# alanross/AlvaAR

Measured on NVIDIA H100. Metric: frames_per_sec_720p_1000orb_20kf_ba, higher is better.
Workload: dtype u8/f64

## Files before the change

alvaar_b200/csrc/ba.cu:

```cuda
#include "alva_common.cuh"
#include "../../include/alva_b200.h"
#include <math.h>
#include <float.h>
#include <string.h>

namespace {

constexpr int NMAX = 128;
constexpr int LIN_THREADS = 128;
constexpr int NBMAX = NMAX / 6;
constexpr int MAXKEYS = NBMAX * (NBMAX + 1) / 2;
constexpr int BS_THREADS = 128;

struct BaState {
    double radius, decrease_factor, x_cost, cand_cost, xnorm, gmax, model_change;
    double se_min, se_cur, se_ref, se_cand, se_acc_ref, se_acc_cand;
    double initial_cost, push_cost;
    int reuse_diagonal, invalid_steps, iteration, last_success, n_success, n_iter, term, done;
    int relin, step_ok, ncols, chol_ok;
    int use_gather, nb, nbad, has_last;
    int skipped, pad0;
};

struct BaProblem {
// ... 722 lines not shown
        double av[4], bv[4];
#pragma unroll
        for (int t = 0; t < 4; t++) { av[t] = __ldg(row + i0 + 8 * t + cc); bv[t] = __ldg(row + j0 + 8 * t + cc); }
#pragma unroll
        for (int a = 0; a < 4; a++)
#pragma unroll
            for (int b = 0; b < 4; b++) dmma_m8n8k4(acc[a][b][0], acc[a][b][1], av[a], bv[b]);
    }
#pragma unroll
    for (int a = 0; a < 4; a++)
#pragma unroll
        for (int b = 0; b < 4; b++) {
            part[warp][8 * a + cc][8 * b + 2 * kr] = acc[a][b][0];
            part[warp][8 * a + cc][8 * b + 2 * kr + 1] = acc[a][b][1];
        }
    __syncthreads();
    for (int t = threadIdx.x; t < 32 * 32; t += 128) {
        const int r = t >> 5, c = t & 31;
        const double v = part[0][r][c] + part[1][r][c] + part[2][r][c] + part[3][r][c];
        if (v != 0.0) atomicAdd(&P.S[(i0 + r) * NMAX + j0 + c], -v);
    }
}


__device__ __forceinline__ void lm_landmark(const BaProblem& P, int l) {
    const int b = P.lm_start[l], e = P.lm_start[l + 1];
    if (e == b) return;
    const int ca = P.pose_col[P.anch_kf[l]];
    const double sce = P.sce[l];
    double ete = P.De[l] * P.De[l], etb = 0, wa[6] = {0, 0, 0, 0, 0, 0};
    for (int i = b; i < e; i++) {
        const int o = P.lm_obs[i];
        const int cp = P.pose_col[P.obs_kf[o]];
        const double e0 = P.Jd[2 * o] * sce, e1 = P.Jd[2 * o + 1] * sce;
        ete += e0 * e0 + e1 * e1;
        etb += e0 * P.res[2 * o] + e1 * P.res[2 * o + 1];
        for (int c = 0; c < 6; c++) {
            if (ca >= 0) wa[c] += (e0 * P.Ja[12 * o + c] + e1 * P.Ja[12 * o + 6 + c]) * P.scf[ca + c];
            P.wp[6 * o + c] = cp >= 0 ? (e0 * -P.Ja[12 * o + c] + e1 * -P.Ja[12 * o + 6 + c]) * P.scf[cp + c] : 0.0;
        }
    }
    P.ete[l] = ete;
    P.etb[l] = etb;
    for (int c = 0; c < 6; c++) P.wa[6 * l + c] = wa[c];
}
__global__ void __launch_bounds__(128) ba_lm_kernel(const BaProblem* __restrict__ probs, BaDims D) {
    const BaProblem P = probs[blockIdx.y];
    if (P.st->done) return;
    const int l = blockIdx.x * 128 + threadIdx.x;
    if (P.st->use_gather) { if (l < D.nlm) lm_landmark(P, l); }
    else if (l < D.nlm) schur_landmark<false>(P, D, l);
}

template <bool TRANSPOSE>
__device__ __forceinline__ void gather_entry(const BaProblem& P, uint64_t en, const double* sci, const double* scj, double* acc,
                                             double* rh) {
    const int l = (int)(en >> 48), su = (int)(en >> 40) & 0xff, sv = (int)(en >> 32) & 0xff;
    const double inv = 1.0 / P.ete[l], etb = P.etb[l];
    const int ou = su ? (int)(en >> 16) & 0xffff : -1, ov = sv ? (int)en & 0xffff : -1;
    double wu[6], wv[6];
#pragma unroll
    for (int c = 0; c < 6; c++) {
        wu[c] = (su ? P.wp[6 * ou + c] : P.wa[6 * l + c]) * inv;
        wv[c] = sv ? P.wp[6 * ov + c] : P.wa[6 * l + c];
    }
#define ACC(a, c) acc[TRANSPOSE ? 6 * (c) + (a) : 6 * (a) + (c)]
#pragma unroll
    for (int a = 0; a < 6; a++)
#pragma unroll
        for (int c = 0; c < 6; c++) ACC(a, c) -= wu[a] * wv[c];
    if (su == 0 && sv == 0) {
        const int ob = P.lm_start[l], oe = P.lm_start[l + 1];
        for (int i = ob; i < oe; i++) {
            const int o = P.lm_obs[i];
            double F0[6], F1[6];
#pragma unroll
            for (int c = 0; c < 6; c++) { F0[c] = P.Ja[12 * o + c] * sci[c]; F1[c] = P.Ja[12 * o + 6 + c] * sci[c]; }
            const double r0 = P.res[2 * o], r1 = P.res[2 * o + 1];
#pragma unroll
            for (int a = 0; a < 6; a++) {
                if (!TRANSPOSE) rh[a] += F0[a] * r0 + F1[a] * r1;
#pragma unroll
                for (int c = 0; c < 6; c++) ACC(a, c) += F0[a] * F0[c] + F1[a] * F1[c];
            }
        }
        if (!TRANSPOSE)
#pragma unroll
            for (int a = 0; a < 6; a++) rh[a] -= wu[a] * etb;
    } else if (su == sv) {
        double F0[6], F1[6];
#pragma unroll
        for (int c = 0; c < 6; c++) { F0[c] = -P.Ja[12 * ou + c] * sci[c]; F1[c] = -P.Ja[12 * ou + 6 + c] * sci[c]; }
        const double r0 = P.res[2 * ou], r1 = P.res[2 * ou + 1];
#pragma unroll
        for (int a = 0; a < 6; a++) {
            if (!TRANSPOSE) rh[a] += F0[a] * r0 + F1[a] * r1 - wu[a] * etb;
#pragma unroll
            for (int c = 0; c < 6; c++) ACC(a, c) += F0[a] * F0[c] + F1[a] * F1[c];
        }
    } else if (su == 0 || sv == 0) {
        const int o = su ? ou : ov;
        double A0[6], A1[6];
#pragma unroll
        for (int a = 0; a < 6; a++) {
            A0[a] = (su ? -P.Ja[12 * o + a] : P.Ja[12 * o + a]) * sci[a];
            A1[a] = (su ? -P.Ja[12 * o + 6 + a] : P.Ja[12 * o + 6 + a]) * sci[a];
        }
#pragma unroll
        for (int c = 0; c < 6; c++) {
            const double b0 = (sv ? -P.Ja[12 * o + c] : P.Ja[12 * o + c]) * scj[c];
            const double b1 = (sv ? -P.Ja[12 * o + 6 + c] : P.Ja[12 * o + 6 + c]) * scj[c];
#pragma unroll
            for (int a = 0; a < 6; a++) ACC(a, c) += A0[a] * b0 + A1[a] * b1;
        }
    }
#undef ACC
}

constexpr int GA_THREADS = 64, GA_SPLIT = 8;
constexpr int GA_GRID = NBMAX * GA_SPLIT + (MAXKEYS - NBMAX);
__global__ void __launch_bounds__(GA_THREADS, 8) ba_gather_kernel(const BaProblem* __restrict__ probs, BaDims D) {
    const BaProblem P = probs[blockIdx.y];
    const BaState& st = *P.st;
    if (st.done || !st.use_gather) return;
    int bi, bj, part = 0, nparts = 1;
    if ((int)blockIdx.x < NBMAX * GA_SPLIT) { bi = bj = blockIdx.x / GA_SPLIT; part = blockIdx.x % GA_SPLIT; nparts = GA_SPLIT; }
    else {
        int rem = blockIdx.x - NBMAX * GA_SPLIT;
        bi = 0;
        while (bi < NBMAX - 1 && rem >= NBMAX - 1 - bi) { rem -= NBMAX - 1 - bi; bi++; }
        bj = bi + 1 + rem;
    }
    if (bi >= st.nb || bj >= st.nb) return;
    const int blk = bi * NBMAX + bj;
    __shared__ double red[GA_THREADS / 32][42];
    __shared__ int last_s;
    const int tid = threadIdx.x, lane = tid & 31, warp = tid >> 5;
    const int ci = 6 * bi, cj = 6 * bj;
    const int eb = P.blk_off[blk], ee = eb + P.blk_start[blk + 1];
    double acc[36], rh[6];
#pragma unroll
    for (int i = 0; i < 36; i++) acc[i] = 0.0;
#pragma unroll
    for (int i = 0; i < 6; i++) rh[i] = 0.0;
    double sci[6], scj[6];
#pragma unroll
    for (int c = 0; c < 6; c++) { sci[c] = P.scf[ci + c]; scj[c] = P.scf[cj + c]; }
    for (int idx = eb + part * GA_THREADS + tid; idx < ee; idx += nparts * GA_THREADS) {
        const uint64_t en = P.pairs[idx];
        gather_entry<false>(P, en, sci, scj, acc, rh);
    }
#pragma unroll
    for (int i = 0; i < 36; i++) {
#pragma unroll
        for (int off = 16; off; off >>= 1) acc[i] += __shfl_xor_sync(0xffffffffu, acc[i], off);
        if (lane == 0) red[warp][i] = acc[i];
    }
#pragma unroll
    for (int i = 0; i < 6; i++) {
#pragma unroll
        for (int off = 16; off; off >>= 1) rh[i] += __shfl_xor_sync(0xffffffffu, rh[i], off);
        if (lane == 0) red[warp][36 + i] = rh[i];
    }
    __syncthreads();
    if (nparts > 1) {
        double* slot = P.ga_part + ((size_t)bi * GA_SPLIT + part) * 42;
        for (int x = tid; x < 42; x += GA_THREADS) {
            double v = 0;
#pragma unroll
            for (int wv = 0; wv < GA_THREADS / 32; wv++) v += red[wv][x];
            slot[x] = v;
        }
        __threadfence();
        __syncthreads();
        if (tid == 0) last_s = atomicInc(reinterpret_cast<unsigned int*>(P.ga_ticket + bi), GA_SPLIT - 1) == GA_SPLIT - 1;
        __syncthreads();
        if (!last_s) return;
        __threadfence();
    }
    for (int x = tid; x < 42; x += GA_THREADS) {
        double v = 0;
        if (nparts > 1) {
            const volatile double* all = P.ga_part + (size_t)bi * GA_SPLIT * 42;
#pragma unroll
            for (int q = 0; q < GA_SPLIT; q++) v += all[q * 42 + x];
        } else {
#pragma unroll
            for (int wv = 0; wv < GA_THREADS / 32; wv++) v += red[wv][x];
        }
        if (x < 36) {
            const int a = x / 6, c = x % 6;
            if (bi == bj) P.S[(ci + a) * NMAX + ci + c] = v + (a == c ? P.Df[ci + a] * P.Df[ci + a] : 0.0);
            else { P.S[(ci + a) * NMAX + cj + c] = v; P.S[(cj + c) * NMAX + ci + a] = v; }
        } else if (bi == bj) P.rhs[ci + x - 36] = v;
    }
}

constexpr int CH_TILES = 32 * 33 / 2, CH_THREADS = (CH_TILES + 31) / 32 * 32;
__device__ void ba_chol_body(const BaProblem& P, double* sm) {
    BaState& st = *P.st;
    const int n = st.ncols, tid = threadIdx.x, lane = tid & 31;
    const int ld = NMAX + 1;
    double* V = sm;
    double* invd = sm + NMAX * ld;
    __shared__ double pcol[4][NMAX];
    __shared__ double dg[4][4];
    __shared__ double pivinv[2][4];
    __shared__ int ok_s;
    int tj = 0, rem = tid;
    while (tj < 32 && rem >= 32 - tj) { rem -= 32 - tj; tj++; }
    const int ti = tj + rem;
    const bool tile = tid < CH_TILES;
    const int r0 = 4 * ti, c0 = 4 * tj;
    double a[4][4];
#pragma unroll
// ... 370 lines not shown
    mix((uint64_t)(uintptr_t)obs_lm); mix((uint64_t)(uintptr_t)obs_uv); mix((uint64_t)(uintptr_t)flags);
    if (key != ctx->ba_table_key) {
        std::string hostbuf(sizeof(BaProblem) * nprob, '\0');
        BaProblem* hp = reinterpret_cast<BaProblem*>(&hostbuf[0]);
        for (int p = 0; p < nprob; p++) {
            BaProblem& P = hp[p];
            P.calib = calib + 4 * (size_t)p; P.poses = poses + 7 * (size_t)nkf * p; P.pose_const = pose_const + (size_t)nkf * p;
            P.invd = invd + (size_t)nlm * p; P.anch_kf = anch_kf + (size_t)nlm * p; P.anch_uv = anch_uv + 2 * (size_t)nlm * p;
            P.obs_kf = obs_kf + (size_t)nobs * p; P.obs_lm = obs_lm + (size_t)nobs * p; P.obs_uv = obs_uv + 2 * (size_t)nobs * p;
            double* d = reinterpret_cast<double*>(ws + tab + per * p);
            auto take = [&](size_t n) { double* r = d; d += n; return r; };
            P.res = take(2 * (size_t)nobs); P.Ja = take(12 * (size_t)nobs); P.Jd = take(2 * (size_t)nobs);
            P.wp = take(6 * (size_t)nobs);
            P.nf = take(NMAX); P.gf = take(NMAX); P.scf = take(NMAX); P.diagf = take(NMAX); P.Df = take(NMAX);
            P.ne = take(nlm); P.ge = take(nlm); P.sce = take(nlm); P.diage = take(nlm); P.De = take(nlm);
            P.ete = take(nlm); P.etb = take(nlm); P.wa = take(6 * (size_t)nlm); P.ye = take(nlm);
            P.S = take((size_t)NMAX * NMAX); P.rhs = take(NMAX); P.yf = take(NMAX);
            P.cand_poses = take(7 * (size_t)nkf); P.cand_invd = take(nlm); P.cost_part = take(nblk);
            P.Wt = g_ba_dense_schur ? take((size_t)((nlm + 3) / 4 * 4) * NMAX) : nullptr;
            P.mc_part = take((size_t)((nlm + BS_THREADS - 1) / BS_THREADS));
            P.ga_part = take((size_t)NBMAX * GA_SPLIT * 42);
            P.last_poses = local ? take(7 * (size_t)nkf) : nullptr;
            P.last_invd = local ? take(nlm) : nullptr;
            uint8_t* b = reinterpret_cast<uint8_t*>(d);
            P.pose_col = reinterpret_cast<int32_t*>(b); b += align_up((size_t)nkf * 4, 8);
            P.lm_start = reinterpret_cast<int32_t*>(b); b += align_up((size_t)(nlm + 1) * 4, 8);
            P.lm_obs = reinterpret_cast<int32_t*>(b); b += align_up((size_t)nobs * 4, 8);
            P.obs_col = reinterpret_cast<int32_t*>(b); b += align_up((size_t)nobs * 4, 8);
            P.anch_col = reinterpret_cast<int32_t*>(b); b += align_up((size_t)nlm * 4, 8);
            P.pstart = reinterpret_cast<int32_t*>(b); b += align_up((size_t)(NBMAX + 1) * 4, 8);
            P.plist = reinterpret_cast<uint32_t*>(b); b += align_up(((size_t)nobs + (size_t)nlm) * 4, 8);
            P.blk_start = reinterpret_cast<int32_t*>(b); b += align_up((size_t)(NBMAX * NBMAX + 1) * 4, 8);
            P.blk_off = reinterpret_cast<int32_t*>(b); b += align_up((size_t)(NBMAX * NBMAX + 1) * 4, 8);
            P.pairs = reinterpret_cast<uint64_t*>(b); b += align_up((size_t)(8 * (size_t)nobs + 2 * (size_t)nlm) * 8, 8);
            P.ga_ticket = reinterpret_cast<int32_t*>(b); b += align_up((size_t)NBMAX * 4, 8);
            P.obs_lm_in = nullptr; P.obs_lm_w = nullptr; P.flags = nullptr;
            if (local) {
                P.obs_lm_in = P.obs_lm;
                P.obs_lm_w = reinterpret_cast<int32_t*>(b); b += align_up((size_t)nobs * 4, 8);
                P.obs_lm = P.obs_lm_w;
                P.flags = flags + (size_t)nobs * p;
            }
            P.st = reinterpret_cast<BaState*>(b);
        }
        ALVA_CUDA(cudaMemcpyAsync(ws, hp, sizeof(BaProblem) * nprob, cudaMemcpyHostToDevice, ctx->stream));
        ALVA_CUDA(cudaStreamSynchronize(ctx->stream));
        ctx->ba_table_key = key;
    }
    *dp_out = reinterpret_cast<const BaProblem*>(ws);
    *D_out = BaDims{nkf, nlm, nobs, nblk, 0.0, 0, (nlm + 3) / 4 * 4, 8 * nobs + 2 * nlm, (nlm + BS_THREADS - 1) / BS_THREADS, 0};
    return 0;
}

static int ba_run_solve(alva_ctx* ctx, const BaProblem* dp, const BaDims& D, int nprob) {
    const bool dense = g_ba_dense_schur != 0;
    const size_t chol_smem = ((size_t)NMAX * (NMAX + 1) + NMAX) * sizeof(double);
    ALVA_CUDA(cudaFuncSetAttribute(ba_chol_kernel, cudaFuncAttributeMaxDynamicSharedMemorySize, (int)chol_smem));
    ba_setup_kernel<<<nprob, SETUP_THREADS, 0, ctx->stream>>>(dp, D);
    ALVA_LAUNCH_CHECK(ctx);
    const dim3 lin_grid(D.nblk, nprob), schur_grid((D.nlm_pad + 127) / 128, nprob), syrk_grid(16, SYRK_KSPLIT, nprob);
    const dim3 key_grid(GA_GRID, nprob), bs_grid(D.nbs, nprob), stats_grid(D.nbs + NBMAX, nprob);
    bool forked = false;
    if (!dense) {
        const dim3 pr_grid(NBMAX, nprob);
        cudaStream_t ps = ctx->stream;
        if (ctx->aux_stream && cudaEventRecord(ctx->aux_fork, ctx->stream) == cudaSuccess &&
            cudaStreamWaitEvent(ctx->aux_stream, ctx->aux_fork, 0) == cudaSuccess) { ps = ctx->aux_stream; forked = true; }
        ba_pairs_kernel<0><<<pr_grid, 32, 0, ps>>>(dp, D);
        ALVA_LAUNCH_CHECK(ctx);
        ba_pairs_kernel<1><<<pr_grid, 32, 0, ps>>>(dp, D);
        ALVA_LAUNCH_CHECK(ctx);
        if (forked) ALVA_CUDA(cudaEventRecord(ctx->aux_join, ps));
    }
    for (int it = 0; it <= D.max_iter; it++) {
        ba_linearize_kernel<true><<<lin_grid, LIN_THREADS, 0, ctx->stream>>>(dp, D);
        ALVA_LAUNCH_CHECK(ctx);
        ba_stats_kernel<<<stats_grid, BS_THREADS, 0, ctx->stream>>>(dp, D);
        ALVA_LAUNCH_CHECK(ctx);
        ba_pre_kernel<<<nprob, g_ba_ctl_threads, 0, ctx->stream>>>(dp, D);
        ALVA_LAUNCH_CHECK(ctx);
        if (it == D.max_iter) {
            if (forked) { ALVA_CUDA(cudaStreamWaitEvent(ctx->stream, ctx->aux_join, 0)); forked = false; }
            break;
        }
        if (dense) {
            ba_schur_kernel<true><<<schur_grid, 128, 0, ctx->stream>>>(dp, D);
            ALVA_LAUNCH_CHECK(ctx);
            ba_syrk_dmma_kernel<<<syrk_grid, 128, 0, ctx->stream>>>(dp, D);
            ALVA_LAUNCH_CHECK(ctx);
        } else {
            if (forked) { ALVA_CUDA(cudaStreamWaitEvent(ctx->stream, ctx->aux_join, 0)); forked = false; }
            ba_lm_kernel<<<schur_grid, 128, 0, ctx->stream>>>(dp, D);
            ALVA_LAUNCH_CHECK(ctx);
            ba_gather_kernel<<<key_grid, GA_THREADS, 0, ctx->stream>>>(dp, D);
            ALVA_LAUNCH_CHECK(ctx);
        }
        ba_chol_kernel<<<nprob, CH_THREADS, chol_smem, ctx->stream>>>(dp, D);
        ALVA_LAUNCH_CHECK(ctx);
        ba_backsub_kernel<<<bs_grid, BS_THREADS, 0, ctx->stream>>>(dp, D);
        ALVA_LAUNCH_CHECK(ctx);
        ba_linearize_kernel<false><<<lin_grid, LIN_THREADS, 0, ctx->stream>>>(dp, D);
        ALVA_LAUNCH_CHECK(ctx);
        ba_post_kernel<<<nprob, g_ba_ctl_threads, 0, ctx->stream>>>(dp, D);
        ALVA_LAUNCH_CHECK(ctx);
    }
    return 0;
}

static bool ba_args_ok(alva_ctx* ctx, int nprob, int nkf, int nlm, int nobs, const void* calib, const void* poses,
                       const void* pose_const, const void* invd, const void* anch_kf, const void* anch_uv, const void* obs_kf,
                       const void* obs_lm, const void* obs_uv, int max_iter) {
    return ctx && nprob >= 1 && nkf >= 1 && nkf <= 256 && nlm >= 1 && nobs >= 1 && calib && poses && pose_const && invd &&
           anch_kf && anch_uv && obs_kf && obs_lm && obs_uv && max_iter >= 0;
}

extern "C" int alva_k_ba_solve(alva_ctx* ctx, int nprob, int nkf, int nlm, int nobs, const double* calib, double* poses,
                               const uint8_t* pose_const, double* invd, const int32_t* anch_kf, const double* anch_uv,
                               const int32_t* obs_kf, const int32_t* obs_lm, const double* obs_uv, double huber_delta,
                               int max_iter, double* summary) { AlvaDeviceGuard guard__(ctx);
    if (!ba_args_ok(ctx, nprob, nkf, nlm, nobs, calib, poses, pose_const, invd, anch_kf, anch_uv, obs_kf, obs_lm, obs_uv, max_iter)) {
        alva_set_error("alva_k_ba_solve: bad argument (need 1 <= nkf <= 256)");
        return ALVA_E_INVALID;
    }
    const BaProblem* dp;
    BaDims D;
    if (int e = ba_prepare(ctx, nprob, nkf, nlm, nobs, calib, poses, pose_const, invd, anch_kf, anch_uv, obs_kf, obs_lm, obs_uv,
                           nullptr, &dp, &D))
        return e;
    D.huber = huber_delta; D.max_iter = max_iter;
    if (int e = ba_run_solve(ctx, dp, D, nprob)) return e;
    if (summary) {
        ba_summary_kernel<<<nprob, 32, 0, ctx->stream>>>(dp, summary);
        ALVA_LAUNCH_CHECK(ctx);
    }
    return 0;
}

extern "C" int alva_k_ba_local(alva_ctx* ctx, int nprob, int nkf, int nlm, int nobs, const double* calib, double* poses,
                               const uint8_t* pose_const, double* invd, const int32_t* anch_kf, const double* anch_uv,
                               const int32_t* obs_kf, const int32_t* obs_lm, const double* obs_uv, double huber_delta,
                               double chi2_thr, int max_iter, int32_t* flags, double* summary) { AlvaDeviceGuard guard__(ctx);
    if (!ba_args_ok(ctx, nprob, nkf, nlm, nobs, calib, poses, pose_const, invd, anch_kf, anch_uv, obs_kf, obs_lm, obs_uv, max_iter) ||
        !flags) {
        alva_set_error("alva_k_ba_local: bad argument (need 1 <= nkf <= 256, flags != NULL)");
        return ALVA_E_INVALID;
    }
    const BaProblem* dp;
    BaDims D;
    if (int e = ba_prepare(ctx, nprob, nkf, nlm, nobs, calib, poses, pose_const, invd, anch_kf, anch_uv, obs_kf, obs_lm, obs_uv,
                           flags, &dp, &D))
        return e;
    D.huber = huber_delta; D.max_iter = max_iter;
    const dim3 obs_grid(D.nblk, nprob);
    ba_local_init_kernel<<<obs_grid, LIN_THREADS, 0, ctx->stream>>>(dp, D);
    ALVA_LAUNCH_CHECK(ctx);
    if (int e = ba_run_solve(ctx, dp, D, nprob)) return e;
    if (summary) { ba_summary_local_kernel<<<nprob, 32, 0, ctx->stream>>>(dp, summary, 0); ALVA_LAUNCH_CHECK(ctx); }
    ba_flag_kernel<1><<<obs_grid, LIN_THREADS, 0, ctx->stream>>>(dp, D, chi2_thr);
    ALVA_LAUNCH_CHECK(ctx);
    D.pass = 1; D.max_iter = 5;
    if (int e = ba_run_solve(ctx, dp, D, nprob)) return e;
    ba_flag_kernel<2><<<obs_grid, LIN_THREADS, 0, ctx->stream>>>(dp, D, chi2_thr);
    ALVA_LAUNCH_CHECK(ctx);
    if (summary) { ba_summary_local_kernel<<<nprob, 32, 0, ctx->stream>>>(dp, summary, 1); ALVA_LAUNCH_CHECK(ctx); }
    return 0;
}

extern "C" int alva_k_ba_linearize(alva_ctx* ctx, int nkf, int nlm, int nobs, const double* calib, const double* poses,
                                   const double* invd, const int32_t* anch_kf, const double* anch_uv, const int32_t* obs_kf,
                                   const int32_t* obs_lm, const double* obs_uv, double huber_delta, double* res, double* Ja,
                                   double* Jp, double* Jd, double* cost_per_obs) { AlvaDeviceGuard guard__(ctx);
    if (!ctx || nobs < 1 || !calib || !poses || !invd || !res || !Ja || !Jp || !Jd || !cost_per_obs) {
        alva_set_error("alva_k_ba_linearize: bad argument");
        return ALVA_E_INVALID;
    }
    (void)nkf; (void)nlm;
    ba_linearize_dump_kernel<<<(nobs + 127) / 128, 128, 0, ctx->stream>>>(calib, poses, invd, anch_kf, anch_uv, obs_kf, obs_lm,
                                                                         obs_uv, nobs, huber_delta, res, Ja, Jp, Jd, cost_per_obs);
    ALVA_LAUNCH_CHECK(ctx);
    return 0;
}

extern int alva_g_knn_qpw;
int alva_g_ba_overlap = 1;

extern int alva_g_frontend_antipodal, alva_g_frontend_variant, alva_g_frontend_prefetch, alva_g_frontend_ctas;
extern int alva_g_knn_mma, alva_g_knn_mma_mode, alva_g_knn_mma_kind;
extern int alva_g_pipeline_graphs, alva_g_ba_lag;
extern "C" int alva_set_option(const char* name, int value) {
    if (name && !strcmp(name, "ba_dense_schur")) { g_ba_dense_schur = value ? 1 : 0; return 0; }
    if (name && !strcmp(name, "ba_ctl_threads") && (value == 256 || value == 512 || value == 1024)) { g_ba_ctl_threads = value; return 0; }
    if (name && !strcmp(name, "frontend_antipodal")) { alva_g_frontend_antipodal = value ? 1 : 0; return 0; }
    if (name && !strcmp(name, "frontend_variant") && (value == 0 || value == 2)) { alva_g_frontend_variant = value; return 0; }
    if (name && !strcmp(name, "frontend_ctas") && (value == 4 || value == 5)) { alva_g_frontend_ctas = value; return 0; }
    if (name && !strcmp(name, "frontend_prefetch")) { alva_g_frontend_prefetch = value ? 1 : 0; return 0; }
    if (name && !strcmp(name, "pipeline_graphs")) { alva_g_pipeline_graphs = value ? 1 : 0; return 0; }
    if (name && !strcmp(name, "pipeline_ba_lag")) { alva_g_ba_lag = value ? 1 : 0; return 0; }
    if (name && !strcmp(name, "pipeline_ba_overlap")) { alva_g_ba_overlap = value ? 1 : 0; return 0; }
    if (name && !strcmp(name, "knn_qpw") && (value == 4 || value == 8)) { alva_g_knn_qpw = value; return 0; }
    if (name && !strcmp(name, "knn_mma") && value >= 0 && value <= 2) { alva_g_knn_mma = value; return 0; }
    if (name && !strcmp(name, "knn_mma_kind") && (value == 0 || value == 1)) { alva_g_knn_mma_kind = value; return 0; }
    if (name && !strcmp(name, "knn_mma_mode") && value >= 0 && value <= 2) { alva_g_knn_mma_mode = value; return 0; }
    alva_set_error("alva_set_option: unknown option");
    return ALVA_E_INVALID;
}
```

alvaar_b200/lib.py:

```python
import ctypes as C
import os

_HERE = os.path.dirname(os.path.abspath(__file__))
ORB_FMA = 1
ORB_IC_ANGLE = 2
ORB_HARRIS = 4


class AlvaError(RuntimeError):
    pass


def lib_path():
    return os.path.join(_HERE, "libalva_b200.so")


_lib = None


def lib():
    global _lib
    if _lib is None:
        p = lib_path()
        if not os.path.exists(p):
# ... 1 lines not shown
                            "(there is no CPU fallback)")
        L = C.CDLL(p)
        vp, i32, i64 = C.c_void_p, C.c_int, C.c_longlong
        L.alva_version.restype = i32
        L.alva_last_error.restype = C.c_char_p
        L.alva_ctx_create.restype = vp
        L.alva_ctx_create.argtypes = [i32, vp]
        L.alva_ctx_destroy.argtypes = [vp]
        L.alva_ctx_sync.argtypes = [vp]
        L.alva_ctx_launches.restype = i64
        L.alva_ctx_launches.argtypes = [vp]
        L.alva_k_gray.argtypes = [vp, vp, vp, i32, i32, i32]
        L.alva_k_pyrdown.argtypes = [vp, vp, vp, i32, i32, i32]
        L.alva_k_fast9.argtypes = [vp, vp, i32, i32, i32, i32, vp, vp, i32, i32]
        L.alva_k_frontend.argtypes = [vp, vp, i32, i32, i32, vp, vp, vp, vp, i32, vp, vp, i32, i32]
        L.alva_set_option.argtypes = [C.c_char_p, i32]
        L.alva_k_retain_best.argtypes = [vp, vp, vp, i32, i32, i32, i32, i32, i32, vp, vp, i32]
        for name, args in _OPTIONAL.items():
            if hasattr(L, name):
                getattr(L, name).argtypes = args
        _lib = L
    return _lib


_vp, _i32 = C.c_void_p, C.c_int
_OPTIONAL = {
    "alva_k_orb_blur": [_vp, _vp, _vp, _i32, _i32, _i32, _i32],
    "alva_k_orb_describe": [_vp, _vp, _vp, _i32, _i32, _i32, _vp, _vp, _i32, _i32, _vp, _vp, _vp],
    "alva_k_hamming_knn2": [_vp, _vp, _i32, _vp, _i32, _vp],
    "alva_k_hamming_knn2_batch": [_vp, _vp, _vp, _i32, _i32, _vp, _i32, _vp],
    "alva_h_frontend": [_vp, _vp, _i32, _i32, _i32, _i32, _vp, _vp, _i32],
    "alva_k_scharr": [_vp, _vp, _vp, _i32, _i32, _i32],
    "alva_k_clahe": [_vp, _vp, _vp, _i32, _i32, _i32, C.c_double, _i32, _i32],
    "alva_k_detect_grid": [_vp, _vp, _i32, _i32, _i32, _i32, _vp, _vp, _i32, _vp, _vp, _vp, _vp, _vp, _i32],
    "alva_k_corner_subpix": [_vp, _vp, _i32, _i32, _i32, _vp, _vp, _i32],
    "alva_k_match_to_map": [_vp, _i32, _i32, _i32, C.c_double, C.c_double, C.c_double, C.c_double, _vp, _i32, _vp, _vp, _i32, _i32, _vp,
                            _i32, _vp, _vp, _vp, _vp, _vp, _vp, _vp, _i32, _vp, C.c_float, C.c_float, _vp, _vp, _vp],
    "alva_k_match_to_map_dist": [_vp, _i32, _i32, _i32, C.c_double, C.c_double, C.c_double, C.c_double, _vp, _i32, _vp, _vp, _i32, _i32,
                                 _vp, _i32, _vp, _vp, _vp, _vp, _vp, _vp, _vp, _i32, _vp, C.c_float, C.c_float, _vp, _vp, _vp, _vp],
    "alva_k_undistort_points": [_vp, _vp, _vp, _i32, _i32, _vp, _vp, _vp],
    "alva_k_project_points": [_vp, _vp, _i32, _vp, _vp, _vp],
    "alva_k_p3p_lmeds": [_vp, _i32, _i32, _vp, _vp, _vp, _i32, C.c_float, C.c_float, C.c_float, C.c_uint32, _vp, _vp, _vp],
    "alva_k_pnp": [_vp, _i32, _i32, _vp, _vp, _vp, _vp, _vp, C.c_double, C.c_double, _i32, _i32, _i32, _vp, _vp],
    "alva_k_essential_5pt": [_vp, _i32, _i32, _vp, _vp, _vp, _i32, C.c_float, _i32, C.c_float, C.c_float, C.c_uint32, _vp, _vp, _vp],
    "alva_k_triangulate": [_vp, _vp, _vp, _vp, _i32, _vp],
    "alva_k_klt_lk": [_vp, _vp, _vp, _vp, _i32, _i32, _i32, _i32, _i32, _i32, _i32, C.c_double, _i32, _vp, _vp, _vp, _i32, _vp, _vp],
    "alva_k_klt_fb": [_vp, _vp, _vp, _vp, _vp, _i32, _i32, _i32, _i32, _i32, _i32, C.c_float, C.c_float, _vp, _vp, _vp, _i32, _vp],
    "alva_k_harris": [_vp, _vp, _i32, _i32, _i32, _vp, _vp, _i32, _vp],
    "alva_k_orb_detect": [_vp, _vp, _i32, _i32, _i32, _i32, _i32, _i32, _vp, _vp, _vp, _i32],
    "alva_k_ba_solve": [_vp, _i32, _i32, _i32, _i32, _vp, _vp, _vp, _vp, _vp, _vp, _vp, _vp, _vp, C.c_double, _i32, _vp],
    "alva_k_ba_local": [_vp, _i32, _i32, _i32, _i32, _vp, _vp, _vp, _vp, _vp, _vp, _vp, _vp, _vp, C.c_double, C.c_double,
                        _i32, _vp, _vp],
    "alva_k_ba_linearize": [_vp, _i32, _i32, _i32, _vp, _vp, _vp, _vp, _vp, _vp, _vp, _vp, C.c_double, _vp, _vp, _vp, _vp, _vp],
}


def key_x(k):
    return (k >> 8) & 0xFFF


def key_y(k):
    return (k >> 20) & 0xFFF


def key_score(k):
    return k & 0xFF


def unpack_keys(keys):
    import numpy as np
    k = np.asarray(keys).astype(np.int64) & 0xFFFFFFFF
    return np.stack([(k >> 8) & 0xFFF, (k >> 20) & 0xFFF, k & 0xFF], -1).astype(np.int32)


def _ptr(t):
    if t is None:
        return None
    return C.c_void_p(t.data_ptr())


def _f64x4(v):
    return (C.c_double * 4)(*[float(x) for x in v])


class Context:

    def __init__(self, device=0, stream=None):
        self.L = lib()
        if stream is not None and int(stream) == 0:
            stream = 1
        h = self.L.alva_ctx_create(int(device), C.c_void_p(int(stream)) if stream is not None else None)
        if not h:
            raise AlvaError(self.L.alva_last_error().decode())
        self.h = C.c_void_p(h)
        self.device = device

    def close(self):
        if getattr(self, "h", None):
            self.L.alva_ctx_destroy(self.h)
            self.h = None

    def __del__(self):
        try:
            self.close()
        except Exception:
            pass
# ... 78 lines not shown
                _ptr(kp_match), _ptr(kp_dist), _ptr(n_match))
        if dist is None:
            self._chk(self.L.alva_k_match_to_map(*args))
        else:
            self._chk(self.L.alva_k_match_to_map_dist(*args, _f64x4(dist)))

    def undistort_points(self, px, counts, nframes, cap, K, dist, unpx):
        self._chk(self.L.alva_k_undistort_points(self.h, _ptr(px), _ptr(counts), nframes, cap, _f64x4(K), _f64x4(dist), _ptr(unpx)))

    def project_points(self, Xc, n, K, dist, uv):
        self._chk(self.L.alva_k_project_points(self.h, _ptr(Xc), n, _f64x4(K), _f64x4(dist), _ptr(uv)))

    def p3p_lmeds(self, nprob, cap, bvs, wpts, counts, Twc_out, outlier, info=None, max_iter=100, err_px=3.0, fx=1.0, fy=1.0,
                  seed=12345):
        self._chk(self.L.alva_k_p3p_lmeds(self.h, nprob, cap, _ptr(bvs), _ptr(wpts), _ptr(counts), max_iter, err_px, fx, fy,
                                          seed, _ptr(Twc_out), _ptr(outlier), _ptr(info)))

    def essential_5pt(self, nprob, cap, bv1, bv2, counts, Rt_out, outlier, info=None, max_iter=100, err_px=3.0, optimize=True,
                      fx=1.0, fy=1.0, seed=12345):
        self._chk(self.L.alva_k_essential_5pt(self.h, nprob, cap, _ptr(bv1), _ptr(bv2), _ptr(counts), max_iter, err_px,
                                              int(optimize), fx, fy, seed, _ptr(Rt_out), _ptr(outlier), _ptr(info)))

    def triangulate(self, Tlr, bvl, bvr, n, out):
        self._chk(self.L.alva_k_triangulate(self.h, _ptr(Tlr), _ptr(bvl), _ptr(bvr), n, _ptr(out)))

    def pnp(self, nprob, cap, K, uv, X, counts, poses, outlier, summary, huber_delta, chi2_thr, max_iter=5, use_robust=True,
            apply_l2=True):
        self._chk(self.L.alva_k_pnp(self.h, nprob, cap, _ptr(K), _ptr(uv), _ptr(X), _ptr(counts), _ptr(poses), huber_delta,
                                    chi2_thr, max_iter, 1 if use_robust else 0, 1 if apply_l2 else 0, _ptr(outlier),
                                    _ptr(summary)))

    def hamming_knn2_batch(self, q, counts, nbatch, qcap, t, nt, out):
        self._chk(self.L.alva_k_hamming_knn2_batch(self.h, _ptr(q), _ptr(counts), nbatch, qcap, _ptr(t), nt, _ptr(out)))

    def harris(self, gray, w, h, nframes, pts, npts_per_frame, npts, resp):
        self._chk(self.L.alva_k_harris(self.h, _ptr(gray), w, h, nframes, _ptr(pts), _ptr(npts_per_frame), npts, _ptr(resp)))

    def orb_detect(self, gray, w, h, nframes, nfeatures, fast_thr, flags, kp_out, desc, counts, out_cap):
        self._chk(self.L.alva_k_orb_detect(self.h, _ptr(gray), w, h, nframes, nfeatures, fast_thr, flags, _ptr(kp_out),
                                           _ptr(desc), _ptr(counts), out_cap))

    def ba_solve(self, nprob, nkf, nlm, nobs, calib, poses, pose_const, invd, anch_kf, anch_uv, obs_kf, obs_lm, obs_uv,
                 huber, max_iter, summary=None):
        self._chk(self.L.alva_k_ba_solve(self.h, nprob, nkf, nlm, nobs, _ptr(calib), _ptr(poses), _ptr(pose_const), _ptr(invd),
                                         _ptr(anch_kf), _ptr(anch_uv), _ptr(obs_kf), _ptr(obs_lm), _ptr(obs_uv), huber,
                                         max_iter, _ptr(summary)))

    def ba_local(self, nprob, nkf, nlm, nobs, calib, poses, pose_const, invd, anch_kf, anch_uv, obs_kf, obs_lm, obs_uv,
                 huber, chi2_thr, max_iter, flags, summary=None):
        self._chk(self.L.alva_k_ba_local(self.h, nprob, nkf, nlm, nobs, _ptr(calib), _ptr(poses), _ptr(pose_const), _ptr(invd),
                                         _ptr(anch_kf), _ptr(anch_uv), _ptr(obs_kf), _ptr(obs_lm), _ptr(obs_uv), huber,
                                         chi2_thr, max_iter, _ptr(flags), _ptr(summary)))

    def ba_linearize(self, nkf, nlm, nobs, calib, poses, invd, anch_kf, anch_uv, obs_kf, obs_lm, obs_uv, huber, res, Ja, Jp,
                     Jd, cost):
        self._chk(self.L.alva_k_ba_linearize(self.h, nkf, nlm, nobs, _ptr(calib), _ptr(poses), _ptr(invd), _ptr(anch_kf),
                                             _ptr(anch_uv), _ptr(obs_kf), _ptr(obs_lm), _ptr(obs_uv), huber, _ptr(res),
                                             _ptr(Ja), _ptr(Jp), _ptr(Jd), _ptr(cost)))
```

include/alva_b200.h:

```cpp
#ifndef ALVA_B200_H
#define ALVA_B200_H
#include <stdint.h>
#include <stddef.h>

#ifdef __cplusplus
extern "C" {
#endif

#define ALVA_OK            0
#define ALVA_E_INVALID    -1
#define ALVA_E_CUDA       -2
#define ALVA_E_CAPACITY   -3
#define ALVA_E_STATE      -4

#define ALVA_KEY_X(k)     (((k) >> 8) & 0xFFFu)
#define ALVA_KEY_Y(k)     (((k) >> 20) & 0xFFFu)
#define ALVA_KEY_SCORE(k) ((k) & 0xFFu)
#define ALVA_MAX_DIM      4095

#define ALVA_ORB_FMA        1
#define ALVA_ORB_HARRIS     4
#define ALVA_ORB_IC_ANGLE   2

typedef struct alva_ctx alva_ctx;
// ... 56 lines not shown
int alva_k_klt_lk(alva_ctx*, const uint8_t* const* prev_img, const int16_t* const* prev_der, const uint8_t* const* cur_img,
                  int w, int h, int nframes, int pyr_levels, int levels, int win, int max_count, double epsilon,
                  int use_initial, const float* pts, float* next, const int32_t* npts_per_frame, int npts,
                  uint8_t* status, float* err);

int alva_k_klt_fb(alva_ctx*, const uint8_t* const* prev_img, const int16_t* const* prev_der, const uint8_t* const* cur_img,
                  const int16_t* const* cur_der, int w, int h, int nframes, int pyr_levels, int levels, int win,
                  float error_value, float max_fb_dist, const float* pts, float* priors, const int32_t* npts_per_frame,
                  int npts, uint8_t* good);

int alva_k_p3p_lmeds(alva_ctx*, int nprob, int cap, const double* bvs, const double* wpts, const int32_t* counts,
                     int max_iter, float err_px, float fx, float fy, uint32_t seed, double* Twc_out, uint8_t* outlier,
                     double* info);

int alva_k_pnp(alva_ctx*, int nprob, int cap, const double* K, const double* uv, const double* X, const int32_t* counts,
               double* poses, double huber_delta, double chi2_thr, int max_iter, int use_robust, int apply_l2,
               uint8_t* outlier, double* summary);

int alva_k_essential_5pt(alva_ctx*, int nprob, int cap, const double* bv1, const double* bv2, const int32_t* counts,
                         int max_iter, float err_px, int optimize, float fx, float fy, uint32_t seed, double* Rt_out,
                         uint8_t* outlier, double* info);

int alva_k_triangulate(alva_ctx*, const double* Tlr, const double* bvl, const double* bvr, int n, double* out);

int alva_k_match_to_map(alva_ctx*, int w, int h, int cell, double fx, double fy, double cx, double cy, const double* Twc_cur,
                        int n_kp, const int32_t* kp_mp, const float* kp_px, int nkp3d, int n_kf, const double* kf_Twc, int n_mp,
                        const double* mp_wpt, const uint8_t* mp_is3d, const int32_t* obs_start, const int32_t* obs_kf,
                        const float* obs_px, const int32_t* desc_start, const uint8_t* desc, int n_local, const int32_t* local_mp,
                        float max_proj_err, float dist_ratio, int32_t* kp_match, float* kp_dist, int32_t* n_match);
int alva_k_match_to_map_dist(alva_ctx*, int w, int h, int cell, double fx, double fy, double cx, double cy, const double* Twc_cur,
                             int n_kp, const int32_t* kp_mp, const float* kp_px, int nkp3d, int n_kf, const double* kf_Twc, int n_mp,
                             const double* mp_wpt, const uint8_t* mp_is3d, const int32_t* obs_start, const int32_t* obs_kf,
                             const float* obs_px, const int32_t* desc_start, const uint8_t* desc, int n_local, const int32_t* local_mp,
                             float max_proj_err, float dist_ratio, int32_t* kp_match, float* kp_dist, int32_t* n_match,
                             const double* dist4);

int alva_k_ba_solve(alva_ctx*, int nprob, int nkf, int nlm, int nobs, const double* calib, double* poses,
                    const uint8_t* pose_const, double* invd, const int32_t* anch_kf, const double* anch_uv,
                    const int32_t* obs_kf, const int32_t* obs_lm, const double* obs_uv, double huber_delta, int max_iter,
                    double* summary);

int alva_k_ba_local(alva_ctx*, int nprob, int nkf, int nlm, int nobs, const double* calib, double* poses,
                    const uint8_t* pose_const, double* invd, const int32_t* anch_kf, const double* anch_uv,
                    const int32_t* obs_kf, const int32_t* obs_lm, const double* obs_uv, double huber_delta, double chi2_thr,
                    int max_iter, int32_t* flags, double* summary);

int alva_set_option(const char* name, int value);
int alva_debug_knn2_mma(alva_ctx*, const uint8_t* q, int nq, const uint8_t* t, int nt, int32_t* out, int32_t* dbg_dev);

int alva_k_ba_linearize(alva_ctx*, int nkf, int nlm, int nobs, const double* calib, const double* poses, const double* invd,
                        const int32_t* anch_kf, const double* anch_uv, const int32_t* obs_kf, const int32_t* obs_lm,
                        const double* obs_uv, double huber_delta, double* res, double* Ja, double* Jp, double* Jd,
                        double* cost_per_obs);

typedef struct alva_pipeline alva_pipeline;
typedef struct alva_pipeline_config {
    int w, h, batch;
    int fast_thr;
    int nfeatures;
    int orb_flags;
    int map_size;
    int kf_interval;
    int ba_nkf, ba_nlm, ba_nobs, ba_max_iter;
    double ba_huber;
    int derivatives;
    int reserved;
} alva_pipeline_config;

alva_pipeline* alva_pipeline_create(alva_ctx*, const alva_pipeline_config*);
void alva_pipeline_destroy(alva_pipeline*);
int  alva_pipeline_set_map(alva_pipeline*, const uint8_t* desc_host, int n);
int  alva_pipeline_set_ba(alva_pipeline*, int slot, const double* calib, const double* poses, const uint8_t* pose_const,
                          const double* invd, const int32_t* anch_kf, const double* anch_uv, const int32_t* obs_kf,
                          const int32_t* obs_lm, const double* obs_uv);
int  alva_pipeline_step_dev(alva_pipeline*, const uint8_t* rgba_dev);
int  alva_pipeline_step_host(alva_pipeline*, const uint8_t* rgba_host, int32_t* nfeat_host, int32_t* matches_host,
                             double* ba_poses_host, double* ba_summary_host);
int  alva_pipeline_submit_host(alva_pipeline*, const uint8_t* rgba_host, int32_t* nfeat_host, int32_t* matches_host,
                               double* ba_poses_host, double* ba_summary_host);
int  alva_pipeline_wait(alva_pipeline*);
int  alva_pipeline_profile(alva_pipeline*, int enable);
int  alva_pipeline_frontend_ms(alva_pipeline*, float* ms, int n);
int  alva_pipeline_info(const alva_pipeline*, int32_t* out4);
int  alva_pipeline_graph_stats(alva_pipeline*, int32_t* out3);
int  alva_pipeline_drain(alva_pipeline*);
void* alva_pipeline_buffer(alva_pipeline*, int which);

alva_system* alva_system_create(int device);
void alva_system_destroy(alva_system*);
int  alva_system_configure(alva_system*, int w, int h, double fx, double fy, double cx, double cy,
                           double k1, double k2, double p1, double p2);
int  alva_system_reset(alva_system*);
int  alva_system_set_clahe(alva_system*, int enabled, double clip_limit, int tile_size);
int  alva_system_set_distortion(alva_system*, double k1, double k2, double p1, double p2);
int  alva_system_find_camera_pose(alva_system*, const uint8_t* rgba, float* pose16);
int  alva_system_find_camera_pose_ts(alva_system*, const uint8_t* rgba, double t_ms, float* pose16);
int  alva_system_find_camera_pose_imu(alva_system*, const uint8_t* rgba, const double* imu, float* pose16);
int  alva_system_find_plane(alva_system*, float* out16, int iterations);
int  alva_system_get_frame_points(alva_system*, int32_t* xy, int cap_pairs);
int  alva_system_num_matched(alva_system*);
int  alva_system_get_tracks(alva_system*, int32_t* ids, float* px, uint8_t* is3d, double* wpt, int cap);
int  alva_system_get_descriptors(alva_system*, uint8_t* desc, uint8_t* has, int cap);
int  alva_system_pin_buffer(alva_system*, void* host_ptr, size_t bytes);
int  alva_system_unpin_buffer(alva_system*, void* host_ptr);
#define ALVA_LC_MAGIC        0x464B4C41
#define ALVA_LC_VERSION      1
// ... 41 lines not shown
```

Measured before the change: 39050.

## Split gather Schur block rows across thread pairs to halve register accumulators

```diff
diff --git a/alvaar_b200/csrc/ba.cu b/alvaar_b200/csrc/ba.cu
--- a/alvaar_b200/csrc/ba.cu
+++ b/alvaar_b200/csrc/ba.cu
@@ -798,74 +798,78 @@
     else if (l < D.nlm) schur_landmark<false>(P, D, l);
 }
 
-template <bool TRANSPOSE>
-__device__ __forceinline__ void gather_entry(const BaProblem& P, uint64_t en, const double* sci, const double* scj, double* acc,
-                                             double* rh) {
+__device__ __forceinline__ void gather_entry(const BaProblem& P, uint64_t en, int a0, const double* sca, const double* scj,
+                                             double* acc, double* rh) {
     const int l = (int)(en >> 48), su = (int)(en >> 40) & 0xff, sv = (int)(en >> 32) & 0xff;
     const double inv = 1.0 / P.ete[l], etb = P.etb[l];
     const int ou = su ? (int)(en >> 16) & 0xffff : -1, ov = sv ? (int)en & 0xffff : -1;
-    double wu[6], wv[6];
+    const double* wup = (su ? P.wp + 6 * ou : P.wa + 6 * l) + a0;
+    const double* wvp = sv ? P.wp + 6 * ov : P.wa + 6 * l;
+    double wu[3];
+#pragma unroll
+    for (int a = 0; a < 3; a++) wu[a] = wup[a] * inv;
 #pragma unroll
     for (int c = 0; c < 6; c++) {
-        wu[c] = (su ? P.wp[6 * ou + c] : P.wa[6 * l + c]) * inv;
-        wv[c] = sv ? P.wp[6 * ov + c] : P.wa[6 * l + c];
-    }
-#define ACC(a, c) acc[TRANSPOSE ? 6 * (c) + (a) : 6 * (a) + (c)]
-#pragma unroll
-    for (int a = 0; a < 6; a++)
-#pragma unroll
-        for (int c = 0; c < 6; c++) ACC(a, c) -= wu[a] * wv[c];
+        const double wv = wvp[c];
+#pragma unroll
+        for (int a = 0; a < 3; a++) acc[6 * a + c] -= wu[a] * wv;
+    }
     if (su == 0 && sv == 0) {
         const int ob = P.lm_start[l], oe = P.lm_start[l + 1];
         for (int i = ob; i < oe; i++) {
-            const int o = P.lm_obs[i];
-            double F0[6], F1[6];
-#pragma unroll
-            for (int c = 0; c < 6; c++) { F0[c] = P.Ja[12 * o + c] * sci[c]; F1[c] = P.Ja[12 * o + 6 + c] * sci[c]; }
-            const double r0 = P.res[2 * o], r1 = P.res[2 * o + 1];
-#pragma unroll
-            for (int a = 0; a < 6; a++) {
-                if (!TRANSPOSE) rh[a] += F0[a] * r0 + F1[a] * r1;
-#pragma unroll
-                for (int c = 0; c < 6; c++) ACC(a, c) += F0[a] * F0[c] + F1[a] * F1[c];
-            }
-        }
-        if (!TRANSPOSE)
-#pragma unroll
-            for (int a = 0; a < 6; a++) rh[a] -= wu[a] * etb;
+            const double* J = P.Ja + 12 * P.lm_obs[i];
+            const double* r = P.res + 2 * P.lm_obs[i];
+            double R0[3], R1[3];
+#pragma unroll
+            for (int a = 0; a < 3; a++) { R0[a] = J[a0 + a] * sca[a]; R1[a] = J[6 + a0 + a] * sca[a]; }
+            const double r0 = r[0], r1 = r[1];
+#pragma unroll
+            for (int a = 0; a < 3; a++) rh[a] += R0[a] * r0 + R1[a] * r1;
+#pragma unroll
+            for (int c = 0; c < 6; c++) {
+                const double f0 = J[c] * scj[c], f1 = J[6 + c] * scj[c];
+#pragma unroll
+                for (int a = 0; a < 3; a++) acc[6 * a + c] += R0[a] * f0 + R1[a] * f1;
+            }
+        }
+#pragma unroll
+        for (int a = 0; a < 3; a++) rh[a] -= wu[a] * etb;
     } else if (su == sv) {
-        double F0[6], F1[6];
-#pragma unroll
-        for (int c = 0; c < 6; c++) { F0[c] = -P.Ja[12 * ou + c] * sci[c]; F1[c] = -P.Ja[12 * ou + 6 + c] * sci[c]; }
+        const double* J = P.Ja + 12 * ou;
+        double R0[3], R1[3];
+#pragma unroll
+        for (int a = 0; a < 3; a++) { R0[a] = -J[a0 + a] * sca[a]; R1[a] = -J[6 + a0 + a] * sca[a]; }
         const double r0 = P.res[2 * ou], r1 = P.res[2 * ou + 1];
 #pragma unroll
-        for (int a = 0; a < 6; a++) {
-            if (!TRANSPOSE) rh[a] += F0[a] * r0 + F1[a] * r1 - wu[a] * etb;
-#pragma unroll
-            for (int c = 0; c < 6; c++) ACC(a, c) += F0[a] * F0[c] + F1[a] * F1[c];
+        for (int a = 0; a < 3; a++) rh[a] += R0[a] * r0 + R1[a] * r1 - wu[a] * etb;
+#pragma unroll
+        for (int c = 0; c < 6; c++) {
+            const double f0 = -J[c] * scj[c], f1 = -J[6 + c] * scj[c];
+#pragma unroll
+            for (int a = 0; a < 3; a++) acc[6 * a + c] += R0[a] * f0 + R1[a] * f1;
         }
     } else if (su == 0 || sv == 0) {
-        const int o = su ? ou : ov;
-        double A0[6], A1[6];
-#pragma unroll
-        for (int a = 0; a < 6; a++) {
-            A0[a] = (su ? -P.Ja[12 * o + a] : P.Ja[12 * o + a]) * sci[a];
-            A1[a] = (su ? -P.Ja[12 * o + 6 + a] : P.Ja[12 * o + 6 + a]) * sci[a];
+        const double* J = P.Ja + 12 * (su ? ou : ov);
+        double A0[3], A1[3];
+#pragma unroll
+        for (int a = 0; a < 3; a++) {
+            A0[a] = (su ? -J[a0 + a] : J[a0 + a]) * sca[a];
+            A1[a] = (su ? -J[6 + a0 + a] : J[6 + a0 + a]) * sca[a];
         }
 #pragma unroll
         for (int c = 0; c < 6; c++) {
-            const double b0 = (sv ? -P.Ja[12 * o + c] : P.Ja[12 * o + c]) * scj[c];
-            const double b1 = (sv ? -P.Ja[12 * o + 6 + c] : P.Ja[12 * o + 6 + c]) * scj[c];
-#pragma unroll
-            for (int a = 0; a < 6; a++) ACC(a, c) += A0[a] * b0 + A1[a] * b1;
-        }
-    }
-#undef ACC
-}
-
-constexpr int GA_THREADS = 64, GA_SPLIT = 8;
+            const double b0 = (sv ? -J[c] : J[c]) * scj[c];
+            const double b1 = (sv ? -J[6 + c] : J[6 + c]) * scj[c];
+#pragma unroll
+            for (int a = 0; a < 3; a++) acc[6 * a + c] += A0[a] * b0 + A1[a] * b1;
+        }
+    }
+}
+
+constexpr int GA_THREADS = 128, GA_SPLIT = 8;
+constexpr int GA_SLOTS = GA_THREADS / 2;
 constexpr int GA_GRID = NBMAX * GA_SPLIT + (MAXKEYS - NBMAX);
-__global__ void __launch_bounds__(GA_THREADS, 8) ba_gather_kernel(const BaProblem* __restrict__ probs, BaDims D) {
+__global__ void __launch_bounds__(GA_THREADS, 5) ba_gather_kernel(const BaProblem* __restrict__ probs, BaDims D) {
     const BaProblem P = probs[blockIdx.y];
     const BaState& st = *P.st;
     if (st.done || !st.use_gather) return;
@@ -882,31 +886,34 @@
     __shared__ double red[GA_THREADS / 32][42];
     __shared__ int last_s;
     const int tid = threadIdx.x, lane = tid & 31, warp = tid >> 5;
+    const int half = tid & 1, a0 = 3 * half;
     const int ci = 6 * bi, cj = 6 * bj;
     const int eb = P.blk_off[blk], ee = eb + P.blk_start[blk + 1];
-    double acc[36], rh[6];
-#pragma unroll
-    for (int i = 0; i < 36; i++) acc[i] = 0.0;
-#pragma unroll
-    for (int i = 0; i < 6; i++) rh[i] = 0.0;
-    double sci[6], scj[6];
-#pragma unroll
-    for (int c = 0; c < 6; c++) { sci[c] = P.scf[ci + c]; scj[c] = P.scf[cj + c]; }
-    for (int idx = eb + part * GA_THREADS + tid; idx < ee; idx += nparts * GA_THREADS) {
+    double acc[18], rh[3];
+#pragma unroll
+    for (int i = 0; i < 18; i++) acc[i] = 0.0;
+#pragma unroll
+    for (int i = 0; i < 3; i++) rh[i] = 0.0;
+    double sca[3], scj[6];
+#pragma unroll
+    for (int a = 0; a < 3; a++) sca[a] = P.scf[ci + a0 + a];
+#pragma unroll
+    for (int c = 0; c < 6; c++) scj[c] = P.scf[cj + c];
+    for (int idx = eb + part * GA_SLOTS + (tid >> 1); idx < ee; idx += nparts * GA_SLOTS) {
         const uint64_t en = P.pairs[idx];
-        gather_entry<false>(P, en, sci, scj, acc, rh);
-    }
-#pragma unroll
-    for (int i = 0; i < 36; i++) {
-#pragma unroll
-        for (int off = 16; off; off >>= 1) acc[i] += __shfl_xor_sync(0xffffffffu, acc[i], off);
-        if (lane == 0) red[warp][i] = acc[i];
-    }
-#pragma unroll
-    for (int i = 0; i < 6; i++) {
-#pragma unroll
-        for (int off = 16; off; off >>= 1) rh[i] += __shfl_xor_sync(0xffffffffu, rh[i], off);
-        if (lane == 0) red[warp][36 + i] = rh[i];
+        gather_entry(P, en, a0, sca, scj, acc, rh);
+    }
+#pragma unroll
+    for (int i = 0; i < 18; i++) {
+#pragma unroll
+        for (int off = 16; off > 1; off >>= 1) acc[i] += __shfl_xor_sync(0xffffffffu, acc[i], off);
+        if (lane < 2) red[warp][6 * a0 + i] = acc[i];
+    }
+#pragma unroll
+    for (int i = 0; i < 3; i++) {
+#pragma unroll
+        for (int off = 16; off > 1; off >>= 1) rh[i] += __shfl_xor_sync(0xffffffffu, rh[i], off);
+        if (lane < 2) red[warp][36 + a0 + i] = rh[i];
     }
     __syncthreads();
     if (nparts > 1) {
@@ -1383,7 +1390,7 @@
     return 0;
 }
 
-static int ba_run_solve(alva_ctx* ctx, const BaProblem* dp, const BaDims& D, int nprob) {
+static int ba_run_solve(alva_ctx* ctx, const BaProblem* dp, const BaDims& D, int nprob, bool schur_only = false) {
     const bool dense = g_ba_dense_schur != 0;
     const size_t chol_smem = ((size_t)NMAX * (NMAX + 1) + NMAX) * sizeof(double);
     ALVA_CUDA(cudaFuncSetAttribute(ba_chol_kernel, cudaFuncAttributeMaxDynamicSharedMemorySize, (int)chol_smem));
@@ -1426,6 +1433,7 @@
             ba_gather_kernel<<<key_grid, GA_THREADS, 0, ctx->stream>>>(dp, D);
             ALVA_LAUNCH_CHECK(ctx);
         }
+        if (schur_only) return 0;
         ba_chol_kernel<<<nprob, CH_THREADS, chol_smem, ctx->stream>>>(dp, D);
         ALVA_LAUNCH_CHECK(ctx);
         ba_backsub_kernel<<<bs_grid, BS_THREADS, 0, ctx->stream>>>(dp, D);
@@ -1497,6 +1505,40 @@
     return 0;
 }
 
+__global__ void ba_schur_dump_kernel(const BaProblem* __restrict__ probs, BaDims D, double* S, double* rhs, double* scf,
+                                     double* Df, double* sce, double* De, int32_t* info) {
+    const BaProblem P = probs[blockIdx.x];
+    const size_t p = blockIdx.x;
+    for (int i = threadIdx.x; i < NMAX * NMAX; i += blockDim.x) S[p * NMAX * NMAX + i] = P.S[i];
+    for (int i = threadIdx.x; i < NMAX; i += blockDim.x) {
+        rhs[p * NMAX + i] = P.rhs[i]; scf[p * NMAX + i] = P.scf[i]; Df[p * NMAX + i] = P.Df[i];
+    }
+    for (int l = threadIdx.x; l < D.nlm; l += blockDim.x) { sce[p * D.nlm + l] = P.sce[l]; De[p * D.nlm + l] = P.De[l]; }
+    if (threadIdx.x == 0) { info[2 * p] = P.st->ncols; info[2 * p + 1] = P.st->use_gather; }
+}
+
+extern "C" int alva_k_ba_schur_dump(alva_ctx* ctx, int nprob, int nkf, int nlm, int nobs, const double* calib, double* poses,
+                                    const uint8_t* pose_const, double* invd, const int32_t* anch_kf, const double* anch_uv,
+                                    const int32_t* obs_kf, const int32_t* obs_lm, const double* obs_uv, double huber_delta,
+                                    double* S, double* rhs, double* scf, double* Df, double* sce, double* De, int32_t* info) {
+    AlvaDeviceGuard guard__(ctx);
+    if (!ba_args_ok(ctx, nprob, nkf, nlm, nobs, calib, poses, pose_const, invd, anch_kf, anch_uv, obs_kf, obs_lm, obs_uv, 1) ||
+        !S || !rhs || !scf || !Df || !sce || !De || !info) {
+        alva_set_error("alva_k_ba_schur_dump: bad argument (need 1 <= nkf <= 256 and every output)");
+        return ALVA_E_INVALID;
+    }
+    const BaProblem* dp;
+    BaDims D;
+    if (int e = ba_prepare(ctx, nprob, nkf, nlm, nobs, calib, poses, pose_const, invd, anch_kf, anch_uv, obs_kf, obs_lm, obs_uv,
+                           nullptr, &dp, &D))
+        return e;
+    D.huber = huber_delta; D.max_iter = 1;
+    if (int e = ba_run_solve(ctx, dp, D, nprob, true)) return e;
+    ba_schur_dump_kernel<<<nprob, 256, 0, ctx->stream>>>(dp, D, S, rhs, scf, Df, sce, De, info);
+    ALVA_LAUNCH_CHECK(ctx);
+    return 0;
+}
+
 extern "C" int alva_k_ba_linearize(alva_ctx* ctx, int nkf, int nlm, int nobs, const double* calib, const double* poses,
                                    const double* invd, const int32_t* anch_kf, const double* anch_uv, const int32_t* obs_kf,
                                    const int32_t* obs_lm, const double* obs_uv, double huber_delta, double* res, double* Ja,
diff --git a/alvaar_b200/lib.py b/alvaar_b200/lib.py
--- a/alvaar_b200/lib.py
+++ b/alvaar_b200/lib.py
@@ -77,6 +77,8 @@
     "alva_k_ba_local": [_vp, _i32, _i32, _i32, _i32, _vp, _vp, _vp, _vp, _vp, _vp, _vp, _vp, _vp, C.c_double, C.c_double,
                         _i32, _vp, _vp],
     "alva_k_ba_linearize": [_vp, _i32, _i32, _i32, _vp, _vp, _vp, _vp, _vp, _vp, _vp, _vp, C.c_double, _vp, _vp, _vp, _vp, _vp],
+    "alva_k_ba_schur_dump": [_vp, _i32, _i32, _i32, _i32, _vp, _vp, _vp, _vp, _vp, _vp, _vp, _vp, _vp, C.c_double, _vp, _vp,
+                             _vp, _vp, _vp, _vp, _vp],
 }
 
 
@@ -261,6 +263,12 @@
                                          _ptr(anch_kf), _ptr(anch_uv), _ptr(obs_kf), _ptr(obs_lm), _ptr(obs_uv), huber,
                                          chi2_thr, max_iter, _ptr(flags), _ptr(summary)))
 
+    def ba_schur_dump(self, nprob, nkf, nlm, nobs, calib, poses, pose_const, invd, anch_kf, anch_uv, obs_kf, obs_lm, obs_uv,
+                      huber, S, rhs, scf, Df, sce, De, info):
+        self._chk(self.L.alva_k_ba_schur_dump(self.h, nprob, nkf, nlm, nobs, _ptr(calib), _ptr(poses), _ptr(pose_const),
+                                              _ptr(invd), _ptr(anch_kf), _ptr(anch_uv), _ptr(obs_kf), _ptr(obs_lm), _ptr(obs_uv),
+                                              huber, _ptr(S), _ptr(rhs), _ptr(scf), _ptr(Df), _ptr(sce), _ptr(De), _ptr(info)))
+
     def ba_linearize(self, nkf, nlm, nobs, calib, poses, invd, anch_kf, anch_uv, obs_kf, obs_lm, obs_uv, huber, res, Ja, Jp,
                      Jd, cost):
         self._chk(self.L.alva_k_ba_linearize(self.h, nkf, nlm, nobs, _ptr(calib), _ptr(poses), _ptr(invd), _ptr(anch_kf),
diff --git a/include/alva_b200.h b/include/alva_b200.h
--- a/include/alva_b200.h
+++ b/include/alva_b200.h
@@ -132,6 +132,10 @@
                         const int32_t* anch_kf, const double* anch_uv, const int32_t* obs_kf, const int32_t* obs_lm,
                         const double* obs_uv, double huber_delta, double* res, double* Ja, double* Jp, double* Jd,
                         double* cost_per_obs);
+int alva_k_ba_schur_dump(alva_ctx*, int nprob, int nkf, int nlm, int nobs, const double* calib, double* poses,
+                         const uint8_t* pose_const, double* invd, const int32_t* anch_kf, const double* anch_uv,
+                         const int32_t* obs_kf, const int32_t* obs_lm, const double* obs_uv, double huber_delta, double* S,
+                         double* rhs, double* scf, double* Df, double* sce, double* De, int32_t* info);
 
 typedef struct alva_pipeline alva_pipeline;
 typedef struct alva_pipeline_config {
```

Measured after the change: 39660 (median of 6 runs). +1.6%, better.
